# fzi-forschungszentrum-informatik/muvo

Measured on AMD Instinct MI355X. Metric: world-model training samples/sec (seq_len=10), higher is better.
Workload: dtype f32 storage/accumulate; large contractions (convolutions, transformer Linear) as bf16x3 split products

## Files before the change

include/muvo_hip.h:

```cpp
#ifndef MUVO_HIP_H
#define MUVO_HIP_H
#include <stdint.h>

#ifdef __cplusplus
extern "C" {
#endif

#define MUVO_OK 0
#define MUVO_ERR_INVALID_ARG (-1)
#define MUVO_ERR_HIP (-2)

#define MUVO_ACT_NONE 0
#define MUVO_ACT_RELU 1
#define MUVO_ACT_LEAKY 2
#define MUVO_ACT_ELU 3
#define MUVO_ACT_TANH 4
#define MUVO_ACT_SIGMOID 5

const char* muvo_last_error(void);
int muvo_abi_version(void);
int muvo_selftest_mfma(void* stream);
int muvo_set_deterministic(int on);
int muvo_reset_accumulators(void);
int muvo_get_deterministic(void);
// ... 9 lines not shown
#define MUVO_CONV_F32 0
#define MUVO_CONV_BF16X3 1
#define MUVO_CONV_MODE_DEFAULT MUVO_CONV_BF16X3
int muvo_conv_set_products(int n);
int muvo_conv_get_products(void);
int muvo_conv_set_mode(int mode);
int muvo_conv_get_mode(void);
int muvo_conv_set_bf16x3_min_gflop(double gflop_per_item);
int muvo_linear_bf16x3_pack_floats(int in_f, int out_f, int64_t* fwd_floats, int64_t* dgrad_floats);
int muvo_linear_bf16x3_pack(int in_f, int out_f, const float* w, float* wp_fwd, float* wp_dgrad, void* stream);
int64_t muvo_linear_bf16x3_workspace_bytes(int64_t rows, int features);
int muvo_linear_bf16x3_split(const float* x, int64_t rows, int features, void* ws, void* stream);
int muvo_linear_bf16x3_forward(int64_t rows, int in_f, int out_f, const void* ws_x, const float* wp_fwd, const float* bias,
                               float* y, int act, float slope, void* stream);
int muvo_linear_bf16x3_dgrad(int64_t rows, int in_f, int out_f, const void* ws_dz, const float* wp_dgrad, float* dx,
                             void* stream);
int muvo_linear_bf16x3_wgrad(int64_t rows, int in_f, int out_f, const void* ws_x, const void* ws_dz, float* scratch,
                             float* dw, void* stream);
int64_t muvo_pack_table_item_bytes(void);
int muvo_conv_pack_table_add(void* host_items, int capacity, int* n_items, int64_t* n_blocks, const muvo_conv_desc* d,
                             const float* w, float* wp_fwd, float* wp_dgrad);
int muvo_linear_bf16x3_pack_table_add(void* host_items, int capacity, int* n_items, int64_t* n_blocks, int in_f, int out_f,
                                      const float* w, float* wp_fwd, float* wp_dgrad);
int muvo_pack_table_run(const void* dev_items, int n_items, int64_t n_blocks, void* stream);
int muvo_conv_pack_sizes(const muvo_conv_desc* d, int64_t* fwd_floats, int64_t* dgrad_floats);
int muvo_conv_pack_weights(const muvo_conv_desc* d, const float* w, float* wp_fwd, float* wp_dgrad, void* stream);
int64_t muvo_conv_workspace_bytes(const muvo_conv_desc* d, int op);
int muvo_conv_kernel_family(const muvo_conv_desc* d, int op);
int muvo_conv_kernel_variant(const muvo_conv_desc* d, int op);
int muvo_conv_forward(const muvo_conv_desc* d, const float* x, const float* wp_fwd, const float* bias, float* y, int act,
                      float slope, void* ws, void* stream);
int muvo_conv_dgrad(const muvo_conv_desc* d, const float* dy, const float* wp_dgrad, float* dx, void* ws, int ws_valid,
                    void* stream);
int muvo_conv_forward_head_supported(const muvo_conv_desc* d, int CO);
int muvo_conv_forward_head(const muvo_conv_desc* d, const float* x, const float* wp_fwd, const float* bias, float* y, int act,
                           float slope, void* ws, const float* head_w, const float* head_b, int CO, float* logits, void* stream);
int muvo_conv_forward_moments_supported(const muvo_conv_desc* d);
int muvo_conv_forward_moments(const muvo_conv_desc* d, const float* x, const float* wp_fwd, const float* bias, float* y, int act,
                              float slope, double* moments, void* stream);
int muvo_adain_fwd_moments(const float* x, const float* style, float* y, float* save_mean, float* save_rstd, double* moments,
                           int N, int C, int64_t S, float eps, void* stream);
int muvo_adain_affine(const float* style, double* moments, float* save_mean, float* save_rstd, float* aff, int N, int C, int64_t S,
                      float eps, void* stream);
int muvo_conv_affine_supported(const muvo_conv_desc* d);
int muvo_conv_forward_affine(const muvo_conv_desc* d, const float* x, const float* aff, const float* wp_fwd, const float* bias,
                             float* y, int act, float slope, double* moments, void* stream);
int muvo_conv_wgrad_affine(const muvo_conv_desc* d, const float* x, const float* aff, const float* dy, float* dw, float* dbias,
                           void* stream);
int muvo_grouped_linear_fwd(const float* x, int M, int K, int L, const float* const* W, const float* const* b, float* const* Y,
                            const int* N, void* stream);
int muvo_grouped_linear_bwd(const float* x, int M, int K, int L, const float* const* W, float* const* dY, float* dx,
                            float* const* dW, float* const* db, const int* N, void* stream);
int muvo_bf3_loop_clock(double* shader_mhz, double* us_per_k_step);
int muvo_adain_head_supported(int C, int CO, int64_t S);
int muvo_adain_head_fwd(const float* x, const float* style, float* save_mean, float* save_rstd, double* moments, const float* head_w,
                        const float* head_b, float* logits, int N, int C, int CO, int64_t S, float eps, void* stream);
int muvo_adain_head_bwd(const float* x, const float* style, const float* save_mean, const float* save_rstd, const float* head_w,
                        const float* dlogits, float* dx, float* dstyle, float* dhead_w, float* dhead_b, double* ws, int N, int C,
                        int CO, int64_t S, int act, float slope, void* stream);
int muvo_conv_dgrad_accumulate(const muvo_conv_desc* d, const float* dy, const float* wp_dgrad, float* dx, void* stream);
int muvo_conv_prepare_dy(const muvo_conv_desc* d, const float* y, const float* dy, int act, float slope, void* ws_dy,
                         float* dbias, void* stream);
int muvo_conv_prepare_dy_head_supported(const muvo_conv_desc* d, int CO);
int muvo_conv_prepare_dy_head(const muvo_conv_desc* d, const float* y, const float* dy, const float* dhead, const float* head_w,
                              int CO, int act, float slope, void* ws_dy, float* dbias, float* dhead_w, float* dhead_b, void* stream);
int64_t muvo_split_planes_bytes(int N, int C, int64_t S);
int muvo_split_planes(const float* x, void* ws, int N, int C, int64_t S, const float* y, int act, float slope, float* dbias,
                      void* stream);
int muvo_conv_wgrad(const muvo_conv_desc* d, const float* x, const float* dy, float* dwp_scratch, float* dw, float* dbias,
                    void* ws_x, void* ws_dy, int flags, void* stream);

int muvo_bias_grad_nchw(const float* dy, float* db, int N, int M, int64_t S, void* stream);

typedef struct muvo_gemm_desc {
  int32_t M, N, K;
  int64_t sam, sak, sbk, sbn, scm;
  int32_t B1, B2;
  int64_t a_b1, a_b2, b_b1, b_b2, c_b1, c_b2;
  float alpha;
  int32_t bias_div;
  int32_t act;
  float slope;
  int32_t mode;
} muvo_gemm_desc;
int muvo_gemm(const muvo_gemm_desc* d, const float* A, const float* B, float* C, const float* bias, void* stream);

int muvo_bn_train_fwd(const float* x, const float* gamma, const float* beta, const float* residual, float* y,
                      float* save_mean, float* save_rstd, float* running_mean, float* running_var, double* ws, int N, int C,
                      int64_t S, float eps, float momentum, int res_mode, int relu, void* stream);
int muvo_bn_train_bwd(const float* x, const float* y, const float* dy, const float* gamma, const float* beta,
                      const float* save_mean, const float* save_rstd, float* dx, float* dres, float* dgamma, float* dbeta,
                      double* ws, int N, int C, int64_t S, int mask_mode, void* stream);
int muvo_adain_fwd(const float* x, const float* style, float* y, float* save_mean, float* save_rstd, double* ws, int N,
                   int C, int64_t S, int64_t x_batch_stride, float eps, void* stream);
int muvo_adain_bwd(const float* x, const float* style, const float* dy, const float* save_mean, const float* save_rstd,
                   float* dx, float* dstyle, double* ws, int N, int C, int64_t S, int64_t x_batch_stride, int act,
                   float slope, void* stream);
int muvo_add_dropout_layernorm_fwd(const float* x, const float* a, const float* gamma, const float* beta, float* y,
                                   float* z, float* mean, float* rstd, int rows, int E, float eps, float p, uint64_t seed,
                                   void* stream);
int muvo_add_dropout_layernorm_bwd(const float* dy, const float* z, const float* mean, const float* rstd,
                                   const float* gamma, float* dx, float* da, float* dgamma, float* dbeta, int rows, int E,
                                   float p, uint64_t seed, void* stream);

int muvo_act_fwd(const float* x, float* y, int64_t n, int act, float slope, void* stream);
int muvo_act_bwd(const float* y, const float* dy, float* dx, int64_t n, int act, float slope, void* stream);
// ... 213 lines not shown
```

muvo_amd/build.py:

```python
import os
import subprocess
import sys
from concurrent.futures import ThreadPoolExecutor

HERE = os.path.dirname(os.path.abspath(__file__))
CSRC = os.path.join(HERE, 'csrc')
LIB = os.path.join(HERE, 'libmuvo_hip.so')
SOURCES = ['abi.hip', 'conv_gemm.hip', 'conv_vox.hip', 'conv_pw.hip', 'conv_bf3.hip', 'gemm.hip', 'norm.hip', 'elementwise.hip', 'losses.hip', 'chamfer.hip', 'metrics.hip', 'bev.hip', 'input.hip', 'augment.hip', 'attention.hip', 'rssm.hip', 'conv_stem.hip', 'voxelize.hip', 'dataset.hip', 'export.hip', 'visualise.hip']
FLAGS = ['--offload-arch=gfx950', '-O3', '-fPIC', '-std=c++17', '-munsafe-fp-atomics', '-Wno-unused-result', '-Wno-unused-value',
         '-ffp-contract=off', '-Rpass-analysis=kernel-resource-usage',
         '-mllvm', '-instcombine-max-copied-from-constant-users=8000',
         ]
NO_PACKED_FP32 = ['-Xclang', '-target-feature', '-Xclang', '-packed-fp32-ops']
PACKED_FP32_OK = {'conv_gemm.hip'}
SCRATCH_ALLOWED = {'rssm_fwd_kernel': 128, 'rssm_bwd_kernel': 128}


def _check_resources(src, stderr):
    import re
    bad, name = [], None
    for line in stderr.splitlines():
        m = re.search(r'remark: Function Name: (\S+)', line)
        if m:
            name = m.group(1)
            continue
        m = re.search(r'remark:\s+ScratchSize \[bytes/lane\]: (\d+)', line)
        if m and name and int(m.group(1)) > 0:
            short = next((k for k in SCRATCH_ALLOWED if k in name), None)
            if short is None or int(m.group(1)) > SCRATCH_ALLOWED[short]:
                bad.append((name, int(m.group(1))))
    return bad


def _check_packed_fp32(obj, src_name):
    import re
    import tempfile
    llvm = os.environ.get('MUVO_LLVM_BIN', '/opt/rocm/lib/llvm/bin')
    with tempfile.TemporaryDirectory() as td:
        co, fat = os.path.join(td, 'dev.co'), os.path.join(td, 'fat.bin')
        r = subprocess.run([os.path.join(llvm, 'llvm-objcopy'), f'--dump-section=.hip_fatbin={fat}', obj], capture_output=True, text=True)
        if r.returncode == 0:
            r = subprocess.run([os.path.join(llvm, 'clang-offload-bundler'), '--type=o', '--unbundle', f'--input={fat}', f'--output={co}',
                                '--targets=hipv4-amdgcn-amd-amdhsa--gfx950'], capture_output=True, text=True)
        if r.returncode != 0 or not os.path.exists(co) or os.path.getsize(co) == 0:
            raise RuntimeError(f'packed-fp32 guard: cannot extract the gfx950 code object of {obj}: {r.stderr[-300:]}')
        d = subprocess.run([os.path.join(llvm, 'llvm-objdump'), '-d', '--mcpu=gfx950', co], capture_output=True, text=True)
        if d.returncode != 0:
            raise RuntimeError(f'packed-fp32 guard: llvm-objdump failed on {obj}: {d.stderr[-300:]}')
    pk = [l for l in d.stdout.splitlines() if re.search(r'\bv_pk_(mul|add|fma)_f32\b', l)]
    if src_name in PACKED_FP32_OK:
        bad = [l for l in pk if 'op_sel' in l]
        if bad:
            raise RuntimeError(f'{src_name} is listed in PACKED_FP32_OK but contains {len(bad)} packed fp32 instructions with op_sel '
                               f'(muvo_amd/build.py), e.g. {bad[0].strip()[:120]}')
    elif pk:
        raise RuntimeError(f'{src_name}: {len(pk)} packed fp32 VALU instructions although the unit is built without them '
                           f'(muvo_amd/build.py: NO_PACKED_FP32 no longer takes effect?), e.g. {pk[0].strip()[:120]}')


def _stale(out, deps):
    if not os.path.exists(out):
# ... 49 lines not shown
```

muvo_amd/csrc/conv_bf3.h:

```cpp
#pragma once
#include "conv_plan.h"

void bf3_finish_phase(ConvPhase& g);
int bf3_pack_phase(const ConvPhase& g, const float* w, float* wp, hipStream_t st);
long bf3_workspace_bytes(int N, int C, long S);
int bf3_split_input(const float* x, void* ws, int N, int C, long S, hipStream_t st, const float* yact = nullptr, int act = 0,
                    float slope = 0.f, float* dbias = nullptr, const float* dhead = nullptr, const float* head_w = nullptr, int CO = 0,
                    float* dhead_w = nullptr, float* dhead_b = nullptr);
int bf3_launch_fwd_phase(const ConvPhase& g, const void* ws, const float* wp, const float* bias, float* out, int act,
                         float slope, hipStream_t st, int ksplit = 1);
void bf3_set_fused_head(const float* w, const float* b, float* out, int co);
void bf3_set_products(int n);
int bf3_get_products();
int bf3_fwd_ksplit(const ConvPhase& g);
int bf3_wgrad_phase(const ConvPhase& g, const void* ws_x, int Cin_total, const void* ws_dz, int Cout_total, float* wg,
                    float* dw, hipStream_t st);
int bf3_split_rows(const float* x, void* ws, long rows, int C, hipStream_t st);
bool bf3_fwd_uses_pp(const ConvPhase& g);
bool bf3_wgrad_uses_pp(const ConvPhase& g);
struct PackItem {
  ConvPhase g;
  const float* w;
  float* dst;
  long blk0;
  int nblk, pad_;
};
int pack_table_launch(const PackItem* dev_items, int n, long n_blocks, hipStream_t st);
```

muvo_amd/csrc/conv_bf3.hip:

```cpp
#include "conv_bf3.h"
#include <type_traits>

typedef __bf16 bf16x8 __attribute__((ext_vector_type(8)));
typedef __bf16 bf16x2 __attribute__((ext_vector_type(2)));
typedef float f32x2 __attribute__((ext_vector_type(2)));

__device__ unsigned long long g_bf3_clock[3];
extern "C" int muvo_bf3_loop_clock(double* shader_mhz, double* us_per_k_step) {
  unsigned long long h[3] = {0, 0, 0};
  if (hipMemcpyFromSymbol(h, HIP_SYMBOL(g_bf3_clock), sizeof(h)) != hipSuccess) return MUVO_ERR_HIP;
  if (h[1] == 0 || h[2] == 0) { *shader_mhz = 0.0; *us_per_k_step = 0.0; return MUVO_OK; }
  *shader_mhz = (double)h[0] / ((double)h[1] / 100.0);
  *us_per_k_step = (double)h[1] / 100.0 / (double)h[2];
  return MUVO_OK;
}

#ifdef MUVO_BF3_STAMPS
__device__ unsigned long long g_bf3_stamps[8 * 16384];
#define BF3_STAMP(slot)                                                                      \
  if (MUVO_BF3_STAMPS != 3 && threadIdx.x == 0 && blockIdx.x < 16384) g_bf3_stamps[blockIdx.x * 8 + (slot)] = __builtin_amdgcn_s_memrealtime()
extern "C" int muvo_debug_bf3_stamps_reset() {
  void* p = nullptr;
  return hipGetSymbolAddress(&p, HIP_SYMBOL(g_bf3_stamps)) == hipSuccess && hipMemset(p, 0, sizeof(unsigned long long) * 8 * 16384) == hipSuccess ? 0 : 1;
}
// ... 1289 lines not shown
int bf3_get_products() { return g_bf3_products; }

template <int BM, int BN, int WM, int WN, int BKC, int NST, bool ONE>
static int bf3_launch_t(const ConvPhase& g, const void* ws, const float* wp, const float* bias, float* out, int act,
                        float slope, hipStream_t st, int ksplit) {
  constexpr size_t lds0 = (size_t)NST * 2 * BKC * (BM + BN) * 16 + 512 + 4 * BM * WN;
  static_assert(lds0 <= 160 * 1024, "LDS budget");
  constexpr size_t HEAD_LDS = NST == 3 ? 4096 : 0;
  const Bf3Head hd = (NST == 3 && ksplit <= 1) ? t_bf3_head : Bf3Head{nullptr, nullptr, nullptr, 0};
  const size_t lds = lds0 + (hd.co > 0 ? HEAD_LDS : 0);
  static_assert(lds0 + HEAD_LDS <= 160 * 1024, "LDS budget with a fused head");
  static bool attr_set = false;
  static const uint4* zero16 = nullptr;
  if (!attr_set) {
    if (hipFuncSetAttribute((const void*)conv_bf3_kernel<BM, BN, WM, WN, BKC, NST, ONE>, hipFuncAttributeMaxDynamicSharedMemorySize,
                            (int)(lds0 + HEAD_LDS)) != hipSuccess ||
        hipGetSymbolAddress((void**)&zero16, HIP_SYMBOL(g_zero16)) != hipSuccess) {
      muvo_set_error("conv_bf3: kernel attribute / symbol setup failed");
      return MUVO_ERR_HIP;
    }
    attr_set = true;
  }
  const long plane_u4 = (long)g.N * g.ID * g.IH * g.IW * (g.Cp / 8);
  dim3 grid(cdiv(g.npix, BN) * cdiv(g.M, BM), ksplit, 1);
  hipLaunchKernelGGL((conv_bf3_kernel<BM, BN, WM, WN, BKC, NST, ONE>), grid, dim3(64 * WM * WN), lds, st, g, (const uint4*)ws, plane_u4,
                     (const uint4*)wp, bias, out, act, slope, zero16, ksplit, hd.w, hd.b, hd.out, hd.co);
  MUVO_CHECK_LAUNCH("conv_bf3_kernel");
  return MUVO_OK;
}
template <int BM, int BN, int WM, int WN, int BKC, int NST>
static int bf3_launch(const ConvPhase& g, const void* ws, const float* wp, const float* bias, float* out, int act,
                      float slope, hipStream_t st, int ksplit = 1) {
  return g_bf3_products == 1 ? bf3_launch_t<BM, BN, WM, WN, BKC, NST, true>(g, ws, wp, bias, out, act, slope, st, ksplit)
                             : bf3_launch_t<BM, BN, WM, WN, BKC, NST, false>(g, ws, wp, bias, out, act, slope, st, ksplit);
}

bool bf3_fwd_uses_pp(const ConvPhase& g) {
  if (g.M <= 64) return false;
  const long big = g.M > 128 ? (long)cdiv(g.npix, 128) * cdiv(g.M, 256) : (long)cdiv(g.npix, 256) * cdiv(g.M, 128);
  static const int min_blocks = getenv("MUVO_BF3_PP_MIN_BLOCKS") ? atoi(getenv("MUVO_BF3_PP_MIN_BLOCKS")) : 128;
  return big >= min_blocks;
}
bool bf3_wgrad_uses_pp(const ConvPhase& g) { return g.M > 128 || (g.M > 64 && g.C > 64); }

int bf3_fwd_ksplit(const ConvPhase& g) {
  if (g.npix <= 0 || bf3_fwd_uses_pp(g) || muvo_det()) return 1;
  static const int tgt = getenv("MUVO_BF3_KSPLIT_BLOCKS") ? atoi(getenv("MUVO_BF3_KSPLIT_BLOCKS")) : 512;
  static const int min_steps = getenv("MUVO_BF3_KSPLIT_MIN_STEPS") ? atoi(getenv("MUVO_BF3_KSPLIT_MIN_STEPS")) : 16;
  const long tiles = (long)cdiv(g.npix, 128) * cdiv(g.M, 64);
  const int nk = g.Kp / 32;
  if (tiles >= 192 || nk < 2 * min_steps) return 1;
  int ks = cdiv(tgt, tiles);
  if (ks > nk / min_steps) ks = nk / min_steps;
  return ks < 1 ? 1 : ks;
}

void bf3_set_fused_head(const float* w, const float* b, float* out, int co) { t_bf3_head = Bf3Head{w, b, out, co}; }

int bf3_launch_fwd_phase(const ConvPhase& g, const void* ws, const float* wp, const float* bias, float* out, int act,
                         float slope, hipStream_t st, int ksplit) {
  if (g.npix <= 0) return MUVO_OK;
  if (ksplit > 1) return bf3_launch<64, 128, 1, 4, 4, 2>(g, ws, wp, nullptr, out, MUVO_ACT_NONE, 0.f, st, ksplit);
  static const int variant = getenv("MUVO_BF3_VARIANT") ? atoi(getenv("MUVO_BF3_VARIANT")) : 0;
  if (variant == 2) {
    if (g.M > 128) return bf3_launch<256, 128, 4, 2, 4, 2>(g, ws, wp, bias, out, act, slope, st);
    if (g.M > 64) return bf3_launch<128, 256, 2, 4, 4, 2>(g, ws, wp, bias, out, act, slope, st);
  }
  if (bf3_fwd_uses_pp(g)) {
    if (g.M > 128) return bf3_launch<256, 128, 4, 2, 4, 3>(g, ws, wp, bias, out, act, slope, st);
    return bf3_launch<128, 256, 2, 4, 4, 3>(g, ws, wp, bias, out, act, slope, st);
  }
  return bf3_launch<64, 128, 1, 4, 4, 2>(g, ws, wp, bias, out, act, slope, st);
}

static int bf3_wgrad_ksplit(long tiles, int nsteps, int tgt, int minst, int slots) {
  if (muvo_det()) return 1;
  int ksplit = cdiv(tgt, tiles);
  if (ksplit > cdiv(nsteps, minst)) ksplit = cdiv(nsteps, minst);
  if (ksplit < 1) ksplit = 1;
  static const int quant = getenv("MUVO_BF3_WGRAD_QUANT") ? atoi(getenv("MUVO_BF3_WGRAD_QUANT")) : 1;
  if (quant && tiles * ksplit < 4L * slots) {
    const int kmax = nsteps / 12 > 1 ? nsteps / 12 : 1;
    double best = 1e30;
    for (int ks = 1; ks <= kmax && tiles * ks <= 8L * slots; ++ks) {
      const int sps = cdiv(nsteps, ks);
      if (cdiv(nsteps, sps) != ks) continue;
      const double cost = (double)cdiv(tiles * ks, slots) * (sps * 1.2 + 12.0);
      if (cost < best - 1e-9) { best = cost; ksplit = ks; }
    }
  }
  return ksplit;
}

static int bf3_wgrad_xcd_order() {
  static const int v = getenv("MUVO_BF3_WGRAD_XCD") ? atoi(getenv("MUVO_BF3_WGRAD_XCD")) : 1;
  return v;
}

template <int BM, int BN, int WM, int WN, bool ONE>
static int bf3_wgrad_pp_launch_t(const ConvPhase& g, const void* ws_x, int Cin_total, const void* ws_dz, int Cout_total,
                                 float* wg, hipStream_t st) {
  constexpr size_t lds = (size_t)3 * 2 * 32 * (BM / 8 + BN / 8) * 16;
  static bool attr_set = false;
  if (!attr_set) {
    if (hipFuncSetAttribute((const void*)conv_bf3_wgrad_pp_kernel<BM, BN, WM, WN, ONE>, hipFuncAttributeMaxDynamicSharedMemorySize,
                            (int)lds) != hipSuccess) {
      muvo_set_error("conv_bf3_wgrad_pp: kernel attribute setup failed");
      return MUVO_ERR_HIP;
    }
    attr_set = true;
  }
  ConvPhase p = g;
  const int xc8 = roundup(Cin_total, 8) / 8, dzc8 = roundup(Cout_total, 8) / 8;
  p.Cp = xc8 * 8;
// ... 96 lines not shown
```

muvo_amd/csrc/conv_gemm.hip:

```cpp
#include "common.h"
#include "conv_vox.h"
#include "conv_pw.h"
#include "conv_plan.h"
#include "conv_bf3.h"

typedef __bf16 wg_bf16x8 __attribute__((ext_vector_type(8)));
__device__ __forceinline__ void wg_split8(const float (&v)[8], wg_bf16x8& hi, wg_bf16x8& lo) {
  typedef __bf16 b2 __attribute__((ext_vector_type(2)));
  typedef float f2 __attribute__((ext_vector_type(2)));
  unsigned h[4], l[4];
#pragma unroll
  for (int p = 0; p < 4; ++p) {
    const b2 hh = __builtin_convertvector((f2){v[2 * p], v[2 * p + 1]}, b2);
    h[p] = __builtin_bit_cast(unsigned, hh);
    const float h0 = __uint_as_float(h[p] << 16), h1 = __uint_as_float(h[p] & 0xffff0000u);
    const b2 ll = __builtin_convertvector((f2){v[2 * p] - h0, v[2 * p + 1] - h1}, b2);
    l[p] = __builtin_bit_cast(unsigned, ll);
  }
  typedef unsigned u4 __attribute__((ext_vector_type(4)));
  hi = __builtin_bit_cast(wg_bf16x8, (u4){h[0], h[1], h[2], h[3]});
  lo = __builtin_bit_cast(wg_bf16x8, (u4){l[0], l[1], l[2], l[3]});
}

template <int BM, int BN, int WM, int WN, int RUN>
// ... 791 lines not shown
}

static bool wgrad_uses_bf3(const ConvPlan& pf);
int64_t muvo_conv_workspace_bytes(const muvo_conv_desc* d, int op) {
  ConvPlan pl;
  if (op >= 2) {
    if (build_plan(d, &pl, 0, false)) return -1;
    if (pw_applicable(d) || vox_wgrad_ok(d) || !wgrad_uses_bf3(pl)) return 0;
    return op == 2 ? bf3_workspace_bytes(d->N, d->Cin, (long)d->in_sz[0] * d->in_sz[1] * d->in_sz[2])
                   : bf3_workspace_bytes(d->N, d->Cout, (long)d->out_sz[0] * d->out_sz[1] * d->out_sz[2]);
  }
  if (build_plan(d, &pl)) return -1;
  const ConvPhase* ph = op == 0 ? pl.fwd : pl.dgr;
  const int nph = op == 0 ? pl.nfwd : pl.ndgr;
  if (pw_applicable(d)) return 0;
  if (op == 0 ? vox_fwd_ok(d) : vox_dgrad_ok(d)) return 0;
  for (int i = 0; i < nph; ++i)
    if (ph[i].bf3) return bf3_workspace_bytes(ph[i].N, ph[i].C, (long)ph[i].ID * ph[i].IH * ph[i].IW);
  return 0;
}

int muvo_conv_kernel_family(const muvo_conv_desc* d, int op) {
  ConvPlan pl;
  if (pw_applicable(d)) return 3;
  if (op == 2) {
    if (build_plan(d, &pl, 0, false)) return -1;
    if (vox_wgrad_ok(d)) return vox_wgrad_uses_bf3(d) ? 4 : 2;
    return wgrad_uses_bf3(pl) ? 1 : 0;
  }
  if (build_plan(d, &pl)) return -1;
  if (op == 0 ? vox_fwd_ok(d) : vox_dgrad_ok(d)) return vox_uses_bf3(d, op) ? 4 : 2;
  const ConvPhase* ph = op == 0 ? pl.fwd : pl.dgr;
  const int nph = op == 0 ? pl.nfwd : pl.ndgr;
  for (int i = 0; i < nph; ++i)
    if (ph[i].bf3) return 1;
  return 0;
}

int muvo_conv_kernel_variant(const muvo_conv_desc* d, int op) {
  if (muvo_conv_kernel_family(d, op) != 1) return 0;
  ConvPlan pl;
  if (op == 2) {
    if (build_plan(d, &pl, 0, true) || !wgrad_uses_bf3(pl)) {
      if (build_plan(d, &pl, 0, false)) return 0;
    }
    return pl.nfwd > 0 && bf3_wgrad_uses_pp(pl.fwd[0]) ? 1 : 0;
  }
  if (build_plan(d, &pl)) return 0;
  const ConvPhase* ph = op == 0 ? pl.fwd : pl.dgr;
  const int nph = op == 0 ? pl.nfwd : pl.ndgr;
  return nph > 0 && bf3_fwd_uses_pp(ph[0]) ? 1 : 0;
}

static int run_phases(const ConvPhase* ph, int nph, const float* in, const float* wp, const float* bias, float* out, int act,
                      float slope, void* ws, hipStream_t st, bool ws_valid = false) {
  bool split_done = ws_valid;
  static const int any_rule = getenv("MUVO_KSPLIT_ANY") ? atoi(getenv("MUVO_KSPLIT_ANY")) : 1;
  bool use_ksplit = nph > 0 && !any_rule, any_ks = false;
  for (int i = 0; i < nph; ++i) {
    use_ksplit = use_ksplit && phase_ksplit(ph[i]) > 1;
    any_ks = any_ks || phase_ksplit(ph[i]) > 1;
  }
  if (any_rule) use_ksplit = any_ks;
  const long out_total = nph > 0 ? (long)ph[0].N * ph[0].out_sN : 0;
  if (use_ksplit && hipMemsetAsync(out, 0, sizeof(float) * out_total, st) != hipSuccess) {
    muvo_set_error("conv: memset of the split-K output failed");
    return MUVO_ERR_HIP;
  }
  for (int i = 0; i < nph; ++i) {
    if (ph[i].bf3 && !split_done) {
      MUVO_CHECK_ARG(ws != nullptr, "conv: this shape runs on the bf16x3 kernel and needs muvo_conv_workspace_bytes() of workspace");
      int rc = bf3_split_input(in, ws, ph[i].N, ph[i].C, (long)ph[i].ID * ph[i].IH * ph[i].IW, st);
      if (rc) return rc;
      split_done = true;
    }
    const int ks_i = phase_ksplit(ph[i]);
    int rc = launch_fwd_phase(ph[i], in, wp, bias, out, act, slope, st, ws, use_ksplit ? (ks_i > 1 ? ks_i : 2) : 1);
    if (rc) return rc;
  }
  if (use_ksplit && (bias != nullptr || act != MUVO_ACT_NONE)) {
    hipLaunchKernelGGL(bias_act_kernel, dim3(ew_grid(out_total)), dim3(256), 0, st, out, bias, ph[0].Msub, (long)ph[0].out_sC,
                       out_total, act, slope);
    MUVO_CHECK_LAUNCH("bias_act_kernel");
  }
  return MUVO_OK;
}

int muvo_conv_forward(const muvo_conv_desc* d, const float* x, const float* wp_fwd, const float* bias, float* y,
                      int act, float slope, void* ws, void* stream) {
  ConvPlan pl;
  int rc = build_plan(d, &pl);
  if (rc) return rc;
  MUVO_CHECK_ARG(x && wp_fwd && y, "conv_forward: null pointer");
  if (pw_applicable(d)) return pw_forward(d, x, wp_fwd, bias, y, act, slope, (hipStream_t)stream);
  if (vox_fwd_ok(d)) return vox_forward(d, x, wp_fwd, bias, y, act, slope, (hipStream_t)stream, vox_uses_bf3(d, 0));
  return run_phases(pl.fwd, pl.nfwd, x, wp_fwd, bias, y, act, slope, ws, (hipStream_t)stream);
}

int muvo_conv_forward_planes(const muvo_conv_desc* d, const float* x, const float* wp_fwd, const float* bias, float* y, int act,
                             float slope, void* ws, int ws_valid, void* stream) {
  if (!ws_valid) return muvo_conv_forward(d, x, wp_fwd, bias, y, act, slope, ws, stream);
  ConvPlan pl;
  int rc = build_plan(d, &pl);
  if (rc) return rc;
  MUVO_CHECK_ARG(wp_fwd && y && ws, "conv_forward_planes: null pointer");
  MUVO_CHECK_ARG(!pw_applicable(d) && !vox_fwd_ok(d), "conv_forward_planes: this shape does not read split planes");
// ... 365 lines not shown
```

muvo_amd/ops.py:

```python
import collections
import contextlib
import ctypes as C
import math
import os
import threading
import weakref

import torch

_HERE = os.path.dirname(os.path.abspath(__file__))
_LIB_PATH = os.environ.get('MUVO_HIP_LIB') or os.path.join(_HERE, 'libmuvo_hip.so')
_lib = None
_lock = threading.Lock()

ACT_NONE, ACT_RELU, ACT_LEAKY, ACT_ELU, ACT_TANH, ACT_SIGMOID = 0, 1, 2, 3, 4, 5


class ConvDesc(C.Structure):
    _fields_ = [('nd', C.c_int32), ('transposed', C.c_int32), ('N', C.c_int32), ('Cin', C.c_int32), ('Cout', C.c_int32),
                ('in_sz', C.c_int32 * 3), ('out_sz', C.c_int32 * 3), ('ksz', C.c_int32 * 3), ('stride', C.c_int32 * 3),
                ('pad', C.c_int32 * 3), ('dil', C.c_int32 * 3)]


class GemmDesc(C.Structure):
    _fields_ = [('M', C.c_int32), ('N', C.c_int32), ('K', C.c_int32),
                ('sam', C.c_int64), ('sak', C.c_int64), ('sbk', C.c_int64), ('sbn', C.c_int64), ('scm', C.c_int64),
                ('B1', C.c_int32), ('B2', C.c_int32),
                ('a_b1', C.c_int64), ('a_b2', C.c_int64), ('b_b1', C.c_int64), ('b_b2', C.c_int64),
                ('c_b1', C.c_int64), ('c_b2', C.c_int64),
                ('alpha', C.c_float), ('bias_div', C.c_int32), ('act', C.c_int32), ('slope', C.c_float),
                ('mode', C.c_int32)]


EXPORTS = [
    'muvo_last_error', 'muvo_abi_version', 'muvo_selftest_mfma', 'muvo_set_deterministic', 'muvo_get_deterministic', 'muvo_reset_accumulators',
    'muvo_conv_set_products', 'muvo_conv_get_products',
    'muvo_conv_set_mode', 'muvo_conv_get_mode', 'muvo_conv_set_bf16x3_min_gflop', 'muvo_conv_pack_sizes', 'muvo_conv_workspace_bytes', 'muvo_conv_kernel_family', 'muvo_conv_kernel_variant', 'muvo_conv_pack_weights', 'muvo_conv_forward', 'muvo_conv_dgrad', 'muvo_conv_prepare_dy', 'muvo_conv_wgrad', 'muvo_bias_grad_nchw',
    'muvo_gemm',
    'muvo_pack_table_item_bytes', 'muvo_conv_pack_table_add', 'muvo_linear_bf16x3_pack_table_add', 'muvo_pack_table_run',
    'muvo_linear_bf16x3_pack_floats', 'muvo_linear_bf16x3_pack', 'muvo_linear_bf16x3_workspace_bytes', 'muvo_linear_bf16x3_split',
    'muvo_linear_bf16x3_forward', 'muvo_linear_bf16x3_dgrad', 'muvo_linear_bf16x3_wgrad',
    'muvo_bn_train_fwd', 'muvo_bn_train_bwd', 'muvo_adain_fwd', 'muvo_adain_bwd',
    'muvo_add_dropout_layernorm_fwd', 'muvo_add_dropout_layernorm_bwd',
    'muvo_act_fwd', 'muvo_act_bwd', 'muvo_dropout', 'muvo_axpby', 'muvo_copy2d', 'muvo_colsum_acc', 'muvo_batchsum',
    'muvo_nchw_to_tokens', 'muvo_tokens_to_nchw', 'muvo_maxpool2d_fwd', 'muvo_maxpool2d_bwd', 'muvo_avgpool_fwd',
    'muvo_avgpool_bwd', 'muvo_upsample3d_x2_fwd', 'muvo_upsample3d_x2_bwd', 'muvo_preprocess_image',
    'muvo_preprocess_route', 'muvo_divide_scalar', 'muvo_resize_bilinear', 'muvo_resize_nearest_f32',
    'muvo_resize_nearest_u8', 'muvo_softmax_dropout_fwd', 'muvo_softmax_dropout_bwd', 'muvo_gru_fwd', 'muvo_gru_bwd',
    'muvo_rssm_sample_fwd', 'muvo_rssm_sample_bwd',
    'muvo_spatial_loss_fwd', 'muvo_spatial_loss_bwd', 'muvo_spatial_loss_masked_fwd', 'muvo_spatial_loss_masked_bwd', 'muvo_voxel_loss_stats_doubles', 'muvo_voxel_loss_coef_floats',
    'muvo_voxel_loss_fwd', 'muvo_voxel_loss_bwd', 'muvo_l1_rows_fwd', 'muvo_l1_rows_bwd', 'muvo_kl_loss_fwd',
    'muvo_kl_loss_bwd', 'muvo_adamw_step', 'muvo_chamfer_loss_ws_doubles', 'muvo_chamfer_loss_fwd', 'muvo_chamfer_loss_bwd',
    'muvo_ssim_frames', 'muvo_sqdiff_frames', 'muvo_chamfer_sums', 'muvo_ssc_counts', 'muvo_seg_confusion', 'muvo_seg_confusion_index',
    'muvo_frustum_cells', 'muvo_frustum_pool_fwd', 'muvo_frustum_pool_bwd', 'muvo_depth_expectation',
    'muvo_resize_bilinear_bwd', 'muvo_softmax_channel_fwd', 'muvo_softmax_channel_bwd',
    'muvo_range_projection', 'muvo_voxel_grid', 'muvo_seg_ce_fwd', 'muvo_seg_ce_bwd', 'muvo_ssim_maps', 'muvo_ssim_bwd',
    'muvo_instance_labels', 'muvo_pixel_augment', 'muvo_preprocess_route_aug',
    'muvo_split_planes_bytes', 'muvo_split_planes', 'muvo_attention_supported', 'muvo_attention_fwd', 'muvo_attention_bwd',
    'muvo_conv_dgrad_accumulate', 'muvo_conv_forward_moments_supported', 'muvo_conv_forward_moments', 'muvo_adain_fwd_moments',
    'muvo_adain_head_supported', 'muvo_adain_head_fwd', 'muvo_adain_head_bwd', 'muvo_bf3_loop_clock',
    'muvo_grouped_linear_fwd', 'muvo_grouped_linear_bwd', 'muvo_conv_prepare_dy_head', 'muvo_conv_prepare_dy_head_supported',
    'muvo_conv_forward_head_supported', 'muvo_conv_forward_head',
    'muvo_adain_affine', 'muvo_conv_affine_supported', 'muvo_conv_forward_affine', 'muvo_conv_wgrad_affine',
    'muvo_fake_allreduce', 'muvo_resize_bilinear_aa', 'muvo_bn_train_fwd_planes', 'muvo_bn_train_bwd_planes', 'muvo_conv_forward_planes',
    'muvo_stem_conv_supported', 'muvo_stem_conv_forward', 'muvo_stem_conv_wgrad',
    'muvo_rssm_supported', 'muvo_rssm_transposed_floats', 'muvo_rssm_scratch_floats', 'muvo_rssm_forward', 'muvo_rssm_backward',
    'muvo_voxelize_scratch_bytes', 'muvo_voxelize_frames',
    'muvo_birdview_decode_frames', 'muvo_label_components_frames', 'muvo_depth_semantic_decode_frames',
    'muvo_range_projection_frames', 'muvo_voxel_grid_frames',
    'muvo_attention_stream_supported', 'muvo_attention_stream_blocks', 'muvo_attention_stream_fwd', 'muvo_attention_stream_bwd',
    'muvo_voxel_rows_scratch_bytes', 'muvo_voxel_rows_logits', 'muvo_voxel_rows_grid', 'muvo_voxel_rows_write', 'muvo_image_u8',
    'muvo_panel_image', 'muvo_panel_logits', 'muvo_panel_labels', 'muvo_panel_fill', 'muvo_panel_bars', 'muvo_panel_scatter',
    'muvo_panel_voxel_top_logits', 'muvo_panel_voxel_top_grid',
]


def lib():
    global _lib
    if _lib is None:
        with _lock:
            if _lib is None:
                if not os.path.exists(_LIB_PATH):
                    raise RuntimeError(f'{_LIB_PATH} not found: build it with `python -m muvo_amd.build` '
                                       '(there is no fallback path)')
                L = C.CDLL(_LIB_PATH)
                L.muvo_last_error.restype = C.c_char_p
                L.muvo_conv_workspace_bytes.restype = C.c_int64
                L.muvo_linear_bf16x3_workspace_bytes.restype = C.c_int64
                L.muvo_pack_table_item_bytes.restype = C.c_int64
                L.muvo_split_planes_bytes.restype = C.c_int64
                L.muvo_rssm_transposed_floats.restype = C.c_int64
                L.muvo_rssm_scratch_floats.restype = C.c_int64
                L.muvo_voxelize_scratch_bytes.restype = C.c_int64
                L.muvo_voxel_rows_scratch_bytes.restype = C.c_int64
                L.muvo_chamfer_loss_ws_doubles.restype = C.c_int64
                for name in EXPORTS:
                    getattr(L, name)
                _lib = L
    return _lib


def _ck(rc):
    if rc != 0:
        msg = lib().muvo_last_error().decode()
        reset_accumulators()
        raise RuntimeError(f'muvo_hip error {rc}: {msg}')


_MOMENT_BUFS = []


def reset_accumulators():
    try:
        if _lib is not None:
            _lib.muvo_reset_accumulators()
        live = []
        for r in _MOMENT_BUFS:
            t = r()
            if t is not None:
                t.zero_()
                live.append(r)
        _MOMENT_BUFS[:] = live
    except Exception:
        pass


def _st():
    return C.c_void_p(torch._C._cuda_getCurrentRawStream(torch.cuda.current_device()))


def _p(t):
    if t is None:
        return C.c_void_p(0)
    assert t.is_cuda and t.is_contiguous(), 'muvo_hip ops need contiguous device tensors'
    return C.c_void_p(t.data_ptr())


def _f(t):
    assert t is None or t.dtype == torch.float32
    return _p(t)


def _i64(v):
    return C.c_int64(int(v))


def _fl(v):
    return C.c_float(float(v))


_weight_epoch = [0]


def bump_weight_epoch():
    _weight_epoch[0] += 1


CONV_F32, CONV_BF16X3, CONV_BF16 = 0, 1, 2


def set_conv_mode(mode, min_gflop=None):
    _ck(lib().muvo_conv_set_mode(CONV_BF16X3 if int(mode) == CONV_BF16 else int(mode)))
    _ck(lib().muvo_conv_set_products(1 if int(mode) == CONV_BF16 else 3))
    if min_gflop is not None:
        _ck(lib().muvo_conv_set_bf16x3_min_gflop(C.c_double(min_gflop)))
    bump_weight_epoch()
    _plan_epoch[0] += 1


def get_conv_mode():
    m = lib().muvo_conv_get_mode()
    return CONV_BF16 if (m == CONV_BF16X3 and lib().muvo_conv_get_products() == 1) else m


_plan_epoch = [0]


def set_deterministic(on=True):
    global GROUPED_LINEAR
    _ck(lib().muvo_set_deterministic(1 if on else 0))
    GROUPED_LINEAR = (not on) and os.environ.get('MUVO_GROUPED_LINEAR', '1') != '0'
    bump_weight_epoch()
    _plan_epoch[0] += 1


def get_deterministic():
    return bool(lib().muvo_get_deterministic())


_join_queued = [False]


def _queue_final_join():
    def cb():
        _join_queued[0] = False
        join_side_streams()
    try:
        torch.autograd.Variable._execution_engine.queue_callback(cb)
        _join_queued[0] = True
    except RuntimeError:
        pass


def grad_of(p):
    if not p.requires_grad:
        return scratch('frozen_grad_dump', p.numel(), p.device).view(-1)[:p.numel()].view(p.shape)
    if _side_streams and not _join_queued[0]:
        _queue_final_join()
    if p.grad is None:
        view = getattr(p, '_muvo_flat_grad', None)
        if view is not None:
            view.zero_()
            p.grad = view
        else:
            p.grad = torch.zeros_like(p)
    return p.grad


_scratch = {}

# ... 2548 lines not shown
```

Before: 26.58.

## Add direct 3x3 bf16x3 conv kernel with LDS input window reuse

Adds a new bf16x3 forward kernel for stride-1 3x3 2D convolutions. It stages a sliding window of input rows in LDS once per channel group and reuses it across all nine taps, instead of gathering an implicit-GEMM B tile per tap. The kernel software-pipelines the weight and window loads against MFMA work, and it caps k-split by channel groups. It is selected by default for every qualifying shape (the shape rule always returns true). The trade-off is large LDS usage and therefore lower occupancy, plus a new untested code path that replaces the tuned kernels for these shapes.

```diff
diff --git a/include/muvo_hip.h b/include/muvo_hip.h
--- a/include/muvo_hip.h
+++ b/include/muvo_hip.h
@@ -85,6 +85,9 @@
 int muvo_grouped_linear_bwd(const float* x, int M, int K, int L, const float* const* W, float* const* dY, float* dx,
                             float* const* dW, float* const* db, const int* N, void* stream);
 int muvo_bf3_loop_clock(double* shader_mhz, double* us_per_k_step);
+int muvo_bf3_set_direct(int mode);
+int64_t muvo_bf3_direct_launches(void);
+int muvo_bf3_direct_plan(const muvo_conv_desc* d, int op, int32_t* out);
 int muvo_adain_head_supported(int C, int CO, int64_t S);
 int muvo_adain_head_fwd(const float* x, const float* style, float* save_mean, float* save_rstd, double* moments, const float* head_w,
                         const float* head_b, float* logits, int N, int C, int CO, int64_t S, float eps, void* stream);
diff --git a/muvo_amd/build.py b/muvo_amd/build.py
--- a/muvo_amd/build.py
+++ b/muvo_amd/build.py
@@ -6,7 +6,7 @@
 HERE = os.path.dirname(os.path.abspath(__file__))
 CSRC = os.path.join(HERE, 'csrc')
 LIB = os.path.join(HERE, 'libmuvo_hip.so')
-SOURCES = ['abi.hip', 'conv_gemm.hip', 'conv_vox.hip', 'conv_pw.hip', 'conv_bf3.hip', 'gemm.hip', 'norm.hip', 'elementwise.hip', 'losses.hip', 'chamfer.hip', 'metrics.hip', 'bev.hip', 'input.hip', 'augment.hip', 'attention.hip', 'rssm.hip', 'conv_stem.hip', 'voxelize.hip', 'dataset.hip', 'export.hip', 'visualise.hip']
+SOURCES = ['abi.hip', 'conv_gemm.hip', 'conv_vox.hip', 'conv_pw.hip', 'conv_bf3.hip', 'conv_bf3_direct.hip', 'gemm.hip', 'norm.hip', 'elementwise.hip', 'losses.hip', 'chamfer.hip', 'metrics.hip', 'bev.hip', 'input.hip', 'augment.hip', 'attention.hip', 'rssm.hip', 'conv_stem.hip', 'voxelize.hip', 'dataset.hip', 'export.hip', 'visualise.hip']
 FLAGS = ['--offload-arch=gfx950', '-O3', '-fPIC', '-std=c++17', '-munsafe-fp-atomics', '-Wno-unused-result', '-Wno-unused-value',
          '-ffp-contract=off', '-Rpass-analysis=kernel-resource-usage',
          '-mllvm', '-instcombine-max-copied-from-constant-users=8000',
diff --git a/muvo_amd/csrc/conv_bf3.h b/muvo_amd/csrc/conv_bf3.h
--- a/muvo_amd/csrc/conv_bf3.h
+++ b/muvo_amd/csrc/conv_bf3.h
@@ -18,6 +18,20 @@
 int bf3_split_rows(const float* x, void* ws, long rows, int C, hipStream_t st);
 bool bf3_fwd_uses_pp(const ConvPhase& g);
 bool bf3_wgrad_uses_pp(const ConvPhase& g);
+struct Bf3DirectPlan {
+  int use;
+  int qualifies;
+  int rs;
+  int entries;
+  int wep;
+  int lds_bytes;
+  int groups;
+};
+constexpr int BF3_DIRECT_MAX_LDS = (2 * 512 + 8 * 394 + 1) * 16 + 1536;
+bool bf3_direct_plan(const ConvPhase& g, Bf3DirectPlan* pl);
+int bf3_direct_ksplit(const ConvPhase& g, int ks);
+int bf3_direct_launch(const ConvPhase& g, const Bf3DirectPlan& p, const void* ws, const float* wp, const float* bias, float* out,
+                      int act, float slope, hipStream_t st, int ksplit);
 struct PackItem {
   ConvPhase g;
   const float* w;
diff --git a/muvo_amd/csrc/conv_bf3.hip b/muvo_amd/csrc/conv_bf3.hip
--- a/muvo_amd/csrc/conv_bf3.hip
+++ b/muvo_amd/csrc/conv_bf3.hip
@@ -1365,6 +1365,8 @@
   if (tiles >= 192 || nk < 2 * min_steps) return 1;
   int ks = cdiv(tgt, tiles);
   if (ks > nk / min_steps) ks = nk / min_steps;
+  Bf3DirectPlan dp;
+  if (bf3_direct_plan(g, &dp)) return bf3_direct_ksplit(g, ks);
   return ks < 1 ? 1 : ks;
 }
 
@@ -1373,6 +1375,8 @@
 int bf3_launch_fwd_phase(const ConvPhase& g, const void* ws, const float* wp, const float* bias, float* out, int act,
                          float slope, hipStream_t st, int ksplit) {
   if (g.npix <= 0) return MUVO_OK;
+  Bf3DirectPlan dp;
+  if (bf3_direct_plan(g, &dp)) return bf3_direct_launch(g, dp, ws, wp, ksplit > 1 ? nullptr : bias, out, ksplit > 1 ? MUVO_ACT_NONE : act, slope, st, ksplit);
   if (ksplit > 1) return bf3_launch<64, 128, 1, 4, 4, 2>(g, ws, wp, nullptr, out, MUVO_ACT_NONE, 0.f, st, ksplit);
   static const int variant = getenv("MUVO_BF3_VARIANT") ? atoi(getenv("MUVO_BF3_VARIANT")) : 0;
   if (variant == 2) {
diff --git a/muvo_amd/csrc/conv_bf3_direct.hip b/muvo_amd/csrc/conv_bf3_direct.hip
--- /dev/null
+++ b/muvo_amd/csrc/conv_bf3_direct.hip
@@ -0,0 +1,283 @@
+#include "conv_bf3.h"
+#include <atomic>
+
+typedef __bf16 bf16x8 __attribute__((ext_vector_type(8)));
+typedef unsigned u32x4 __attribute__((ext_vector_type(4)));
+
+namespace {
+constexpr int D_BM = 64, D_BN = 128, D_TM = 2, D_TN = 1;
+constexpr int D_ASTAGE = 2 * 4 * D_BM;
+constexpr int D_NPW = 7;
+constexpr int D_TAIL = 512 + 4 * D_BM * 4;
+}
+
+static int g_direct_mode = -1;
+static std::atomic<long long> g_direct_launches{0};
+
+template <bool ONE>
+__global__ void __launch_bounds__(256)
+conv_bf3_direct_kernel(const ConvPhase g, const uint4* __restrict__ xs, long plane_u4, const uint4* __restrict__ wp,
+                       const float* __restrict__ bias, float* __restrict__ out, int act, float slope, int rs, int wep, int ksplit,
+                       int atomic) {
+  constexpr int BM = D_BM, BN = D_BN, TM = D_TM, TN = D_TN, AST = D_ASTAGE, NPW = D_NPW;
+  extern __shared__ uint4 smem[];
+  const int tid = threadIdx.x, lane = tid & 63;
+  const int wave = __builtin_amdgcn_readfirstlane(tid >> 6);
+  uint4* win = smem + 2 * AST;
+  const int ZS = 8 * wep;
+  int* taptab = (int*)(win + ZS + 1);
+  float* sbias = (float*)(taptab + 128) + wave * (32 * TM);
+
+  const int gx = (g.npix + BN - 1) / BN;
+  const int wg = xcd_swizzle(blockIdx.x, gridDim.x);
+  const int bx = wg % gx, by = wg / gx;
+  const int p0 = bx * BN, m_tile = by * BM;
+  const int IW = g.IW, IH = g.IH;
+  const bool runs = IW > 128;
+  const int WE = 2 * rs + 130;
+  const int cp8 = g.Cp >> 3, Mp = g.Mp;
+
+  if (tid < 9) {
+    const int d = g.tap_d[tid];
+    const int ry = ((d >> 8) & 255) - 128 + g.ib[1], rx = (d & 255) - 128 + g.ib[2];
+    taptab[tid] = (ry + 1) * rs + rx + 1;
+    taptab[64 + tid] = (ry + 1) * 4 + rx + 1;
+  }
+  if (tid == 0) win[ZS] = make_uint4(0u, 0u, 0u, 0u);
+  __syncthreads();
+
+  const int pl = wave * 32 + (lane & 31);
+  unsigned vmask = 0u;
+  {
+    const int p = p0 + pl;
+    const bool pv = p < g.npix;
+    int n, iz, iy, ix;
+    decode_pix(g, pv ? p : 0, n, iz, iy, ix);
+#pragma unroll
+    for (int t = 0; t < 9; ++t) {
+      const int d = taptab[64 + t];
+      const bool ok = pv && (unsigned)(iy + (d >> 2) - 1) < (unsigned)IH && (unsigned)(ix + (d & 3) - 1) < (unsigned)IW;
+      vmask |= (unsigned)ok << t;
+    }
+  }
+  int tb[9];
+#pragma unroll
+  for (int t = 0; t < 9; ++t) tb[t] = __builtin_amdgcn_readfirstlane(taptab[t]);
+  const int bl0 = pl + (lane >> 5) * wep;
+
+  const int ng = cp8 >> 2;
+  const int cg0 = (int)blockIdx.y * ng / ksplit, cg1 = ((int)blockIdx.y + 1) * ng / ksplit;
+  if (cg0 >= cg1) return;
+
+  const uint4* wpb = wp + g.wp_off / 4 + m_tile;
+  const __amdgpu_buffer_rsrc_t rs_w = __builtin_amdgcn_make_buffer_rsrc(
+      (void*)wpb, 0, (int)(((long)(g.Kp >> 5) * 8 * g.Mp - m_tile) * 16), 0x00020000);
+  const __amdgpu_buffer_rsrc_t rs_x = __builtin_amdgcn_make_buffer_rsrc((void*)xs, 0, (int)(2 * plane_u4 * 16), 0x00020000);
+  constexpr int OOB = 0x7ffffff0;
+
+  const int npw = (4 * WE + 255) >> 8;
+  int woff[NPW], wl[NPW];
+#pragma unroll
+  for (int q = 0; q < NPW; ++q) {
+    const int item = q * 256 + tid, e = item >> 2, c = item & 3;
+    int qin;
+    if (runs) { const int r = e / 130; qin = p0 + (r - 1) * IW - 1 + (e - r * 130); }
+    else qin = p0 - IW - 1 + e;
+    const bool in_win = e < WE;
+    woff[q] = (in_win && qin >= 0 && qin < g.npix) ? (qin * cp8 + c) * 16 : -1;
+    wl[q] = in_win ? c * wep + e : -1;
+  }
+  u32x4 W[NPW][2];
+  auto wload = [&](int q, int cg) {
+    if (q < npw) {
+      const int goff = cg * 64;
+      const bool ok = woff[q] >= 0 && cg < cg1;
+      W[q][0] = __builtin_bit_cast(u32x4, __builtin_amdgcn_raw_buffer_load_b128(rs_x, ok ? woff[q] + goff : OOB, 0, 0));
+      if constexpr (!ONE)
+        W[q][1] = __builtin_bit_cast(u32x4, __builtin_amdgcn_raw_buffer_load_b128(rs_x, ok ? woff[q] + goff + (int)plane_u4 * 16 : OOB, 0, 0));
+    }
+  };
+  auto wstore = [&](int q) {
+    if (q < npw && wl[q] >= 0) {
+      *(u32x4*)(win + wl[q]) = W[q][0];
+      if constexpr (!ONE) *(u32x4*)(win + 4 * wep + wl[q]) = W[q][1];
+    }
+  };
+  u32x4 RA[2];
+  auto aload = [&](int kt) {
+#pragma unroll
+    for (int q = 0; q < 2; ++q) {
+      const int pc = wave * 2 + q;
+      RA[q] = __builtin_bit_cast(u32x4, __builtin_amdgcn_raw_buffer_load_b128(rs_w, (ONE && pc >= 4) ? OOB : lane * 16, ((kt * 8 + pc) * Mp) * 16, 0));
+    }
+  };
+  auto astore = [&](int stage) {
+#pragma unroll
+    for (int q = 0; q < 2; ++q) *(u32x4*)(smem + stage * AST + (wave * 2 + q) * BM + lane) = RA[q];
+  };
+
+  f32x16 acc[TM][TN];
+#pragma unroll
+  for (int i = 0; i < TM; ++i)
+#pragma unroll
+    for (int r = 0; r < 16; ++r) acc[i][0][r] = 0.f;
+
+  bf16x8 a0h[TM], a0l[TM], b0h, b0l, a1h[TM], a1l[TM], b1h, b1l;
+  auto load_a = [&](int stage, int ks, bf16x8 (&ah)[TM], bf16x8 (&al)[TM]) {
+    const uint4* S = smem + stage * AST + (lane & 31) + (ks * 2 + (lane >> 5)) * BM;
+#pragma unroll
+    for (int i = 0; i < TM; ++i) {
+      ah[i] = __builtin_bit_cast(bf16x8, S[i * 32]);
+      al[i] = __builtin_bit_cast(bf16x8, S[4 * BM + i * 32]);
+    }
+  };
+  auto load_b = [&](int t, int ks, bf16x8& bh, bf16x8& bl) {
+    const bool ok = (vmask >> t) & 1u;
+    const int e = bl0 + tb[t] + ks * 2 * wep;
+    bh = __builtin_bit_cast(bf16x8, win[ok ? e : ZS]);
+    bl = __builtin_bit_cast(bf16x8, win[ok ? e + 4 * wep : ZS]);
+  };
+  auto mma = [&](const bf16x8 (&ah)[TM], const bf16x8 (&al)[TM], const bf16x8& bh, const bf16x8& bl) {
+#pragma unroll
+    for (int i = 0; i < TM; ++i) {
+      if constexpr (!ONE) {
+        acc[i][0] = __builtin_amdgcn_mfma_f32_32x32x16_bf16(al[i], bh, acc[i][0], 0, 0, 0);
+        acc[i][0] = __builtin_amdgcn_mfma_f32_32x32x16_bf16(ah[i], bl, acc[i][0], 0, 0, 0);
+      }
+      acc[i][0] = __builtin_amdgcn_mfma_f32_32x32x16_bf16(ah[i], bh, acc[i][0], 0, 0, 0);
+    }
+  };
+
+  const int kt0 = cg0 * 9;
+#pragma unroll
+  for (int q = 0; q < NPW; ++q) wload(q, cg0);
+  aload(kt0);
+  astore(0);
+#pragma unroll
+  for (int q = 0; q < NPW; ++q) wstore(q);
+  aload(kt0 + 1);
+  astore(1);
+  aload(kt0 + 2);
+  __syncthreads();
+  load_a(0, 0, a0h, a0l);
+  load_b(0, 0, b0h, b0l);
+  __builtin_amdgcn_s_waitcnt(0xC07F);
+
+  int P = 0;
+  for (int cg = cg0; cg < cg1; ++cg) {
+    const bool more = cg + 1 < cg1;
+#pragma unroll
+    for (int t = 0; t < 9; ++t) {
+      const int kt = cg * 9 + t;
+      load_a(P, 1, a1h, a1l);
+      load_b(t, 1, b1h, b1l);
+      __builtin_amdgcn_sched_barrier(0);
+      mma(a0h, a0l, b0h, b0l);
+      __builtin_amdgcn_sched_barrier(0);
+      __builtin_amdgcn_s_waitcnt(0xC07F);
+      __builtin_amdgcn_s_barrier();
+      __builtin_amdgcn_sched_barrier(0);
+      if (t < 8) {
+        load_a(P ^ 1, 0, a0h, a0l);
+        load_b(t + 1, 0, b0h, b0l);
+      }
+      astore(P);
+      aload(kt + 3);
+      if (t < NPW) wload(t, cg + 1);
+      if (t == 8 && more) {
+#pragma unroll
+        for (int q = 0; q < NPW; ++q) wstore(q);
+      }
+      __builtin_amdgcn_sched_barrier(0);
+      mma(a1h, a1l, b1h, b1l);
+      __builtin_amdgcn_sched_barrier(0);
+      __builtin_amdgcn_s_waitcnt(0xC07F);
+      if (t == 8 && more) {
+        __builtin_amdgcn_s_barrier();
+        __builtin_amdgcn_sched_barrier(0);
+        load_a(P ^ 1, 0, a0h, a0l);
+        load_b(0, 0, b0h, b0l);
+        __builtin_amdgcn_s_waitcnt(0xC07F);
+      }
+      P ^= 1;
+    }
+  }
+
+#define BF3D_STORE(ACT) conv_tile_store<ACT, true, true>(g, acc, bias, out, slope, p0, m_tile, 0, wave, lane, sbias, nullptr, 0, nullptr, nullptr)
+  if (atomic) conv_tile_atomic<true>(g, acc, out, p0, m_tile, 0, wave, lane);
+  else { MUVO_ACT_SWITCH(act, BF3D_STORE) }
+}
+
+static int direct_switch() {
+  static const int env = getenv("MUVO_BF3_DIRECT") ? atoi(getenv("MUVO_BF3_DIRECT")) : -1;
+  return g_direct_mode >= 0 ? g_direct_mode : env;
+}
+
+static bool bf3_direct_shape_rule(const ConvPhase& g) {
+  (void)g;
+  return true;
+}
+
+bool bf3_direct_plan(const ConvPhase& g, Bf3DirectPlan* pl) {
+  Bf3DirectPlan p = {};
+  bool ok = g.T == 9 && g.ID == 1 && g.SD == 1 && g.nmerge == 1 && (g.Cp & 31) == 0 && g.Cp >= 32 && g.Kp == 9 * g.Cp &&
+            g.is[0] == 1 && g.is[1] == 1 && g.is[2] == 1 && g.SH == g.IH && g.SW == g.IW && g.npix > 0 &&
+            (long)g.npix == (long)g.N * g.IH * g.IW && !bf3_fwd_uses_pp(g);
+  for (int t = 0; ok && t < 9; ++t) {
+    const int ry = ((g.tap_d[t] >> 8) & 255) - 128 + g.ib[1], rx = (g.tap_d[t] & 255) - 128 + g.ib[2];
+    ok = (((g.tap_d[t] >> 16) & 255) - 128 + g.ib[0]) == 0 && ry >= -1 && ry <= 1 && rx >= -1 && rx <= 1;
+  }
+  p.qualifies = ok ? 1 : 0;
+  if (ok) {
+    p.rs = g.IW > 128 ? 130 : g.IW;
+    p.entries = 2 * p.rs + 130;
+    p.wep = p.entries + ((2 - p.entries) & 7);
+    p.lds_bytes = (2 * D_ASTAGE + 8 * p.wep + 1) * 16 + D_TAIL;
+    p.groups = g.Cp / 32;
+    const int sw = direct_switch();
+    p.use = sw == 0 ? 0 : sw == 1 ? 1 : bf3_direct_shape_rule(g) ? 1 : 0;
+  }
+  *pl = p;
+  return p.use != 0;
+}
+
+int bf3_direct_ksplit(const ConvPhase& g, int ks) {
+  const int ng = g.Cp / 32;
+  if (ks > ng / 2) ks = ng / 2;
+  return ks < 1 ? 1 : ks;
+}
+
+template <bool ONE>
+static int direct_launch_t(const ConvPhase& g, const Bf3DirectPlan& p, const void* ws, const float* wp, const float* bias, float* out,
+                           int act, float slope, hipStream_t st, int ksplit) {
+  static bool attr_set = false;
+  if (!attr_set) {
+    if (hipFuncSetAttribute((const void*)conv_bf3_direct_kernel<ONE>, hipFuncAttributeMaxDynamicSharedMemorySize,
+                            BF3_DIRECT_MAX_LDS) != hipSuccess) {
+      muvo_set_error("conv_bf3_direct: kernel attribute setup failed");
+      return MUVO_ERR_HIP;
+    }
+    attr_set = true;
+  }
+  MUVO_CHECK_ARG(p.lds_bytes <= BF3_DIRECT_MAX_LDS, "conv_bf3_direct: window of %d entries exceeds the LDS budget", p.entries);
+  const long plane_u4 = (long)g.N * g.ID * g.IH * g.IW * (g.Cp / 8);
+  const int ky = ksplit < 1 ? 1 : ksplit > p.groups ? p.groups : ksplit;
+  dim3 grid(cdiv(g.npix, D_BN) * cdiv(g.M, D_BM), ky, 1);
+  hipLaunchKernelGGL((conv_bf3_direct_kernel<ONE>), grid, dim3(256), (size_t)p.lds_bytes, st, g, (const uint4*)ws, plane_u4,
+                     (const uint4*)wp, bias, out, act, slope, p.rs, p.wep, ky, ksplit > 1 ? 1 : 0);
+  MUVO_CHECK_LAUNCH("conv_bf3_direct_kernel");
+  g_direct_launches.fetch_add(1, std::memory_order_relaxed);
+  return MUVO_OK;
+}
+
+int bf3_direct_launch(const ConvPhase& g, const Bf3DirectPlan& p, const void* ws, const float* wp, const float* bias, float* out,
+                      int act, float slope, hipStream_t st, int ksplit) {
+  return bf3_get_products() == 1 ? direct_launch_t<true>(g, p, ws, wp, bias, out, act, slope, st, ksplit)
+                                 : direct_launch_t<false>(g, p, ws, wp, bias, out, act, slope, st, ksplit);
+}
+
+extern "C" int muvo_bf3_set_direct(int mode) {
+  g_direct_mode = mode < 0 ? -1 : mode ? 1 : 0;
+  return MUVO_OK;
+}
+extern "C" int64_t muvo_bf3_direct_launches(void) { return (int64_t)g_direct_launches.load(std::memory_order_relaxed); }
diff --git a/muvo_amd/csrc/conv_gemm.hip b/muvo_amd/csrc/conv_gemm.hip
--- a/muvo_amd/csrc/conv_gemm.hip
+++ b/muvo_amd/csrc/conv_gemm.hip
@@ -867,6 +867,24 @@
   return nph > 0 && bf3_fwd_uses_pp(ph[0]) ? 1 : 0;
 }
 
+int muvo_bf3_direct_plan(const muvo_conv_desc* d, int op, int32_t* out) {
+  MUVO_CHECK_ARG(d && out && (op == 0 || op == 1), "bf3_direct_plan: null pointer or op not 0 / 1");
+  for (int i = 0; i < 10; ++i) out[i] = 0;
+  ConvPlan pl;
+  int rc = build_plan(d, &pl);
+  if (rc) return rc;
+  if (pw_applicable(d) || (op == 0 ? vox_fwd_ok(d) : vox_dgrad_ok(d))) return MUVO_OK;
+  const ConvPhase* ph = op == 0 ? pl.fwd : pl.dgr;
+  const int nph = op == 0 ? pl.nfwd : pl.ndgr;
+  if (nph != 1 || !ph[0].bf3) return MUVO_OK;
+  Bf3DirectPlan p;
+  bf3_direct_plan(ph[0], &p);
+  const int ks = phase_ksplit(ph[0]);
+  out[0] = p.use; out[1] = p.qualifies; out[2] = p.rs; out[3] = p.entries; out[4] = p.wep; out[5] = p.lds_bytes;
+  out[6] = BF3_DIRECT_MAX_LDS; out[7] = p.groups; out[8] = ks; out[9] = ph[0].Kp / 32;
+  return MUVO_OK;
+}
+
 static int run_phases(const ConvPhase* ph, int nph, const float* in, const float* wp, const float* bias, float* out, int act,
                       float slope, void* ws, hipStream_t st, bool ws_valid = false) {
   bool split_done = ws_valid;
diff --git a/muvo_amd/ops.py b/muvo_amd/ops.py
--- a/muvo_amd/ops.py
+++ b/muvo_amd/ops.py
@@ -59,6 +59,7 @@
     'muvo_split_planes_bytes', 'muvo_split_planes', 'muvo_attention_supported', 'muvo_attention_fwd', 'muvo_attention_bwd',
     'muvo_conv_dgrad_accumulate', 'muvo_conv_forward_moments_supported', 'muvo_conv_forward_moments', 'muvo_adain_fwd_moments',
     'muvo_adain_head_supported', 'muvo_adain_head_fwd', 'muvo_adain_head_bwd', 'muvo_bf3_loop_clock',
+    'muvo_bf3_set_direct', 'muvo_bf3_direct_launches', 'muvo_bf3_direct_plan',
     'muvo_grouped_linear_fwd', 'muvo_grouped_linear_bwd', 'muvo_conv_prepare_dy_head', 'muvo_conv_prepare_dy_head_supported',
     'muvo_conv_forward_head_supported', 'muvo_conv_forward_head',
     'muvo_adain_affine', 'muvo_conv_affine_supported', 'muvo_conv_forward_affine', 'muvo_conv_wgrad_affine',
@@ -94,6 +95,7 @@
                 L.muvo_voxelize_scratch_bytes.restype = C.c_int64
                 L.muvo_voxel_rows_scratch_bytes.restype = C.c_int64
                 L.muvo_chamfer_loss_ws_doubles.restype = C.c_int64
+                L.muvo_bf3_direct_launches.restype = C.c_int64
                 for name in EXPORTS:
                     getattr(L, name)
                 _lib = L
@@ -166,6 +168,22 @@
         _ck(lib().muvo_conv_set_bf16x3_min_gflop(C.c_double(min_gflop)))
     bump_weight_epoch()
     _plan_epoch[0] += 1
+
+
+def set_bf3_direct(mode):
+    _ck(lib().muvo_bf3_set_direct(int(mode)))
+    _plan_epoch[0] += 1
+
+
+def bf3_direct_launches():
+    return int(lib().muvo_bf3_direct_launches())
+
+
+def bf3_direct_plan(desc, op=0):
+    out = (C.c_int32 * 10)()
+    _ck(lib().muvo_bf3_direct_plan(C.byref(desc), int(op), out))
+    keys = ('use', 'qualifies', 'rs', 'entries', 'wep', 'lds_bytes', 'lds_max', 'groups', 'ksplit', 'ksteps')
+    return dict(zip(keys, (int(v) for v in out)))
 
 
 def get_conv_mode():
```

Measured after the change: 26.80, median of 6. About the same (+0.8%).
